# MrTornado24/IDE-3D

Measured on AMD Instinct MI355X. Metric: 512x512 RGB+seg frames/s @96 depth samples (whole job), higher is better.
Workload: dtype f32 (3x3 convs + MLPs: fp32 operands as 3 bf16 pieces, 6 products, f32 accumulate)

## Files before the change

### ide-3d_amd/csrc/modconv.hip

```cpp
#include "common.h"
#include "knobs.h"
#include <stdlib.h>
#include <string.h>
#include <type_traits>

namespace ide3d {

typedef float f32x16 __attribute__((ext_vector_type(16)));

#ifdef IDE3D_MC_TRACE
__device__ unsigned long long g_mc_dbg[256];
#define IDE3D_MC_TS(k) { const unsigned long long now_ = __builtin_readcyclecounter(); mc_acc[k] += now_ - mc_last; mc_last = now_; }
#else
#define IDE3D_MC_TS(k)
#endif

enum { MODE_CONV3 = 0, MODE_CONV1 = 1, MODE_TCONV3 = 2, MODE_TCONV3A = 3, MODE_CONV3S2 = 4 };

template <int MODE> struct ModeCfg;
template <> struct ModeCfg<MODE_CONV3>  { static constexpr int KC = 4, WTAPS = 9, MAXT = 9; };
template <> struct ModeCfg<MODE_CONV1>  { static constexpr int KC = 16, WTAPS = 1, MAXT = 1; };
template <> struct ModeCfg<MODE_CONV3S2> { static constexpr int KC = 4, WTAPS = 9, MAXT = 9; };
template <> struct ModeCfg<MODE_TCONV3> { static constexpr int KC = 4, WTAPS = 9, MAXT = 4; };
template <> struct ModeCfg<MODE_TCONV3A> { static constexpr int KC = 4, WTAPS = 9, MAXT = 9; };

template <int MODE, int BIG, int TI, int PH, int PW, int NWV = 4, int KCO = 0>
struct McCfg {
    static constexpr int NT = 64 * NWV;
    static constexpr int BN = TI * PH * PW;
    static_assert(BN == 64 || BN == 128 || BN == 256, "pixel tile must hold 64, 128 or 256 pixels");
    static constexpr int NCLS = (MODE == MODE_TCONV3A) ? 4 : 1;
    using MC = ModeCfg<MODE>;
    static constexpr int KC = KCO ? KCO : MC::KC, WTAPS = MC::WTAPS, MAXT = MC::MAXT;
    static constexpr int WM = BIG ? 2 : 1, WN = NWV / WM;
    static constexpr int MTW = (BIG == 1) ? 2 : 1;
    static constexpr int NTW = (BN / 32) / WN;
    static constexpr int BM = WM * MTW * 32;
    static constexpr int STRIDE = (MODE == MODE_CONV3S2) ? 2 : 1;
    static constexpr int HALO = (MODE == MODE_CONV1 || MODE == MODE_CONV3S2) ? 0 : 1;
    static constexpr int HP = (MODE == MODE_CONV3S2) ? 2 * PH + 1 : PH + 2 * HALO;
    static constexpr int HW = (MODE == MODE_CONV3S2) ? 2 * PW + 1 : PW + 2 * HALO;
    static constexpr int XW = (MODE == MODE_CONV1) ? PW : (MODE == MODE_CONV3S2) ? ((HW + 3) & ~3) : ((PW == 16) ? 48 : HW + 2);
    static constexpr int XS = HP * XW;
    static constexpr int XI = KC * XS;
    static constexpr int LDS_W = MAXT * KC * BM;
    static constexpr int LDS_X = TI * XI;
    static constexpr int NW4 = (LDS_W / 4 + NT - 1) / NT;
    static constexpr int VW = (MODE == MODE_CONV1 && PH == 1 && PW % 4 == 0) ? 4 : 1;
    static constexpr int NXE = (TI * KC * HP * HW / VW + NT - 1) / NT;
};

template <int N>
__device__ __forceinline__ int sel(const int (&a)[N], int t) {
    int v = a[0];
#pragma unroll
    for (int i = 1; i < N; ++i) v = (t == i) ? a[i] : v;
    return v;
}

__host__ __device__ inline int mc_bm(int cout) { return cout > 96 ? 128 : (cout > 32 ? 64 : 32); }
__host__ __device__ inline int mc_kc(int k) { return k == 3 ? 4 : 16; }

__global__ void __launch_bounds__(256)
modconv_pack_kernel(const float* __restrict__ w, int64_t w_batch_stride, int nbatch, int cout, int cin, int taps, int bm, int kc,
                    int mblocks, int cchunks, float* __restrict__ out) {
    const int64_t total = (int64_t)nbatch * mblocks * cchunks * taps * kc * bm;
    const int64_t stride = (int64_t)gridDim.x * blockDim.x;
    for (int64_t i = (int64_t)blockIdx.x * blockDim.x + threadIdx.x; i < total; i += stride) {
        int64_t r = i;
        const int co_l = (int)(r % bm); r /= bm;
        const int cil = (int)(r % kc); r /= kc;
        const int tap = (int)(r % taps); r /= taps;
        const int cc = (int)(r % cchunks); r /= cchunks;
        const int mb = (int)(r % mblocks); r /= mblocks;
        const int nb = (int)r;
        const int co = mb * bm + co_l, ci = cc * kc + cil;
        out[i] = (co < cout && ci < cin) ? w[nb * w_batch_stride + ((int64_t)co * cin + ci) * taps + tap] : 0.f;
    }
}

struct ConvGeom {
    int tiles_x[4], tiles_y[4];
    int tile_base[5];
    int img_groups;
    int mblocks, cchunks, split_k, chunks_per_split;
    int oh, ow;
    int debug;
};

template <int OFF_BYTES>
__device__ __forceinline__ float lds_read_async(unsigned addr) {
    float v;
    asm volatile("ds_read_b32 %0, %1 offset:%2" : "=v"(v) : "v"(addr), "n"(OFF_BYTES));
    return v;
}
template <int PENDING>
__device__ __forceinline__ void lds_wait(float& first) { asm volatile("s_waitcnt lgkmcnt(%1)" : "+v"(first) : "n"(PENDING)); }
__device__ __forceinline__ void lds_pin(float& v) { asm volatile("" : "+v"(v)); }
__device__ __forceinline__ unsigned lds_addr(const float* p) { return (unsigned)(size_t)p; }

template <class F, int... Is>
__device__ __forceinline__ void static_for_impl(F&& f, std::integer_sequence<int, Is...>) { (f(std::integral_constant<int, Is>{}), ...); }
template <int N, class F>
__device__ __forceinline__ void static_for(F&& f) { static_for_impl(f, std::make_integer_sequence<int, N>{}); }

template <int MODE, int XW>
__host__ __device__ constexpr int tap_patch_offset(int t) {
    return (MODE == MODE_CONV1) ? 0
         : (MODE == MODE_TCONV3A) ? ((t / 3 == 2) ? 0 : 1) * XW + ((t % 3 == 2) ? 0 : 1)
         : (t / 3) * XW + (t % 3);
}
template <int MODE>
__host__ __device__ constexpr int tap_class(int t) { return (MODE == MODE_TCONV3A) ? ((t / 3) & 1) * 2 + ((t % 3) & 1) : 0; }

__device__ __forceinline__ void amax_acc(float& m, float v) { m = fmaxf(m, fabsf(v)); }
__device__ __forceinline__ void amax_commit(float* y_amax, int n, float v, bool) {
    if (v > 0.f) amax_raise(y_amax, n, v);
}

template <int MODE, int TI, int PH, int PW, int NWV, int NCLS, int MTW, int NTW, int BM, int SCRATCH, int ROWPAR = -1>
__device__ __forceinline__ void modconv_finish(const ide3d_modconv_params& p, float* __restrict__ partial, const ConvGeom& g,
                                               f32x16 (&acc)[NCLS][MTW][NTW], float* s_w, int mb, int n0, int y0, int x0, int split, int cls,
                                               int wm, int wn, int lp, const float* __restrict__ row_unscale = nullptr, float x_unscale = 1.f,
                                               int team_tid = -1, float* amax_scratch = nullptr) {
    constexpr int NT = 64 * NWV;
    const int tid = team_tid >= 0 ? team_tid : (int)threadIdx.x, lane = tid & 63, wid = tid >> 6, half = lane >> 5;
    const int cpy = cls >> 1, cpx = cls & 1;
    const bool raw = (g.split_k > 1);
    float* const s_dm = s_w;
    float* const s_bi = s_w + TI * BM;
    for (int e = tid; e < TI * BM; e += NT) {
        const int rl = e % BM, co = mb * BM + rl, n = min(n0 + e / BM, p.n - 1);
        float d = (!raw && p.dcoefs && co < p.cout) ? p.dcoefs[(int64_t)n * p.cout + co] : 1.f;
        if (row_unscale) d *= row_unscale[co] * x_unscale;
        s_dm[e] = d;
        if (e < BM) s_bi[e] = (!raw && p.bias && co < p.cout) ? p.bias[co] : 0.f;
    }
    __syncthreads();
    float* const dst = raw ? partial + (int64_t)split * p.n * p.cout * g.oh * g.ow : p.y;
    const int64_t pitch = (!raw && p.y_pitch > 0) ? p.y_pitch : g.ow;
    const float e_alpha = (!raw && p.act == 3) ? p.alpha : 1.f, e_gain = raw ? 1.f : p.gain;
    const float e_clamp = (!raw && p.clamp >= 0.f) ? p.clamp : __builtin_inff();
    const float e_nstr = (!raw && p.noise) ? p.noise_strength : 0.f;
    auto finish = [&](float v, float d, float nz, float bb) {
        v *= d; v += nz; v += bb;
        v = (v > 0.f) ? v : v * e_alpha;
        v *= e_gain;
        return fminf(fmaxf(v, -e_clamp), e_clamp);
    };
    const bool want_amax = !raw && p.y_amax != nullptr;
    float amax_tile = 0.f;
    constexpr int QX = (MODE == MODE_TCONV3A) ? 2 : 1, QY = NCLS / QX;
    static_assert(ROWPAR < 0 || (MODE == MODE_TCONV3A && NCLS == 2), "one row parity = two column classes");
    constexpr int TW = 32 * QX, TP = TW + 8;
    constexpr int AVAIL = SCRATCH - (TI + 1) * BM;
    constexpr int RR = (MODE == MODE_TCONV3 || PW % 4 != 0) ? 0 : (AVAIL >= NWV * 32 * TP) ? 32 : (AVAIL >= NWV * 16 * TP) ? 16 : (AVAIL >= NWV * 8 * TP) ? 8 : 0;
    if constexpr (RR > 0) {
        typedef float f32x4u __attribute__((ext_vector_type(4), aligned(4)));
        float* const T = s_w + (TI + 1) * BM + wid * (RR * TP);
#pragma unroll
        for (int qy = 0; qy < QY; ++qy)
#pragma unroll
        for (int j = 0; j < NTW; ++j) {
            const int pbase = (wn * NTW + j) * 32;
            const int c4 = lane % (TW / 4), row0 = lane / (TW / 4);
            const int pix = pbase + (c4 * 4) / QX, ti = pix / (PH * PW), rem = pix % (PH * PW);
            const int n = n0 + ti, gy = y0 + rem / PW, gx = x0 + rem % PW;
            const int oy = (MODE == MODE_TCONV3A) ? 2 * gy + (ROWPAR >= 0 ? ROWPAR : qy) : gy, ox = (MODE == MODE_TCONV3A) ? 2 * gx : gx;
            const bool px_ok = n < p.n && oy < g.oh && ox < g.ow, full = ox + 3 < g.ow;
            const int64_t pofs = (int64_t)oy * pitch + ox, nofs = (int64_t)oy * g.ow + ox;
            f32x4u nz = {0.f, 0.f, 0.f, 0.f};
            if (e_nstr != 0.f && px_ok) {
                if (full) nz = *reinterpret_cast<const f32x4u*>(p.noise + nofs) * e_nstr;
                else for (int e = 0; e < 4; ++e) if (ox + e < g.ow) nz[e] = p.noise[nofs + e] * e_nstr;
            }
            float* const o_px = dst + (int64_t)n * p.cout * ((int64_t)g.oh * pitch) + pofs;
            float amax_j = 0.f;
#pragma unroll
            for (int i = 0; i < MTW; ++i)
#pragma unroll
            for (int g0 = 0; g0 < 4; g0 += RR / 8) {
#pragma unroll
                for (int qx = 0; qx < QX; ++qx)
#pragma unroll
                    for (int gg = 0; gg < RR / 8; ++gg)
#pragma unroll
                        for (int rr = 0; rr < 4; ++rr)
                            T[(gg * 8 + rr + 4 * half) * TP + lp * QX + qx] = acc[qy * QX + qx][i][j][(g0 + gg) * 4 + rr];
#pragma unroll
                for (int k = 0; k < RR * (TW / 4) / 64; ++k) {
                    const int rowl = row0 + k * (256 / TW);
                    f32x4u v4 = *reinterpret_cast<const f32x4u*>(T + rowl * TP + c4 * 4);
                    const int rl = (wm * MTW + i) * 32 + g0 * 8 + rowl, co = mb * BM + rl;
                    if (!px_ok || co >= p.cout) continue;
                    const float d = s_dm[ti * BM + rl], bb = s_bi[rl];
#pragma unroll
                    for (int e = 0; e < 4; ++e) v4[e] = finish(v4[e], d, nz[e], bb);
                    float* o = o_px + (int64_t)co * ((int64_t)g.oh * pitch);
                    if (full) {
                        *reinterpret_cast<f32x4u*>(o) = v4;
                        if (want_amax) { amax_acc(amax_j, v4[0]); amax_acc(amax_j, v4[1]); amax_acc(amax_j, v4[2]); amax_acc(amax_j, v4[3]); }
                    } else for (int e = 0; e < 4; ++e) if (ox + e < g.ow) { o[e] = v4[e]; amax_acc(amax_j, v4[e]); }
                }
            }
            if (want_amax) { if (TI == 1) amax_tile = fmaxf(amax_tile, amax_j); else if (px_ok) amax_commit(p.y_amax, n, amax_j, false); }
        }
    } else {
#pragma unroll
    for (int q = 0; q < NCLS; ++q)
#pragma unroll
    for (int j = 0; j < NTW; ++j) {
        const int pix = (wn * NTW + j) * 32 + lp;
        const int ti = pix / (PH * PW), rem = pix % (PH * PW);
        const int n = n0 + ti;
        const int gy = y0 + rem / PW, gx = x0 + rem % PW;
        const int oy = (MODE == MODE_TCONV3) ? 2 * gy + cpy : gy, ox = (MODE == MODE_TCONV3) ? 2 * gx + cpx : gx;
        const bool ok = n < p.n && oy < g.oh && ox < g.ow;
        if (!ok) continue;
        const float nz = (e_nstr != 0.f) ? p.noise[oy * g.ow + ox] * e_nstr : 0.f;
        float amax_j = 0.f;
#pragma unroll
        for (int i = 0; i < MTW; ++i)
#pragma unroll
            for (int r = 0; r < 16; ++r) {
                const int rl = (wm * MTW + i) * 32 + (r & 3) + 8 * (r >> 2) + 4 * half;
                const int co = mb * BM + rl;
                if (co >= p.cout) continue;
                const float v = finish(acc[q][i][j][r], s_dm[ti * BM + rl], nz, s_bi[rl]);
                *(dst + (((int64_t)n * p.cout + co) * g.oh + oy) * pitch + ox) = v;
                amax_acc(amax_j, v);
            }
        if (want_amax) { if (TI == 1) amax_tile = fmaxf(amax_tile, amax_j); else amax_commit(p.y_amax, n, amax_j, false); }
    }
    }
    if (TI == 1 && p.y_amax != nullptr && !raw && n0 < p.n)
        amax_raise_block(p.y_amax, n0, amax_tile, amax_scratch ? amax_scratch : s_w);
}

template <int MODE, int BIG, int TI, int PH, int PW, int NWV, int KCO>
__device__ __forceinline__ void modconv_tile(const ide3d_modconv_params& p, const float* __restrict__ wp, float* __restrict__ partial,
                                             const ConvGeom& g, float* s_w, float* s_x, int mb, int tl, int grp, int split, int cls,
                                             int tiles_x) {
    using K = McCfg<MODE, BIG, TI, PH, PW, NWV, KCO>;
#ifdef IDE3D_MC_TRACE
    const unsigned long long mc_t0 = __builtin_readcyclecounter();
#endif
    const int tid = threadIdx.x, lane = tid & 63, wid = tid >> 6;
    const int wm = wid / K::WN, wn = wid % K::WN;
    const int half = lane >> 5, l32 = lane & 31;
    const int txi = tl % tiles_x, tyi = tl / tiles_x;
    const int y0 = tyi * PH, x0 = txi * PW;
    const int n0 = grp * TI;
    const int cpy = cls >> 1, cpx = cls & 1;

    int ntaps, t_widx[K::MAXT], t_off[K::MAXT];
    if (MODE == MODE_CONV3 || MODE == MODE_CONV3S2) {
        ntaps = 9;
#pragma unroll
        for (int t = 0; t < 9; ++t) { t_widx[t] = t; t_off[t] = (t / 3) * K::XW + (t % 3); }
    } else if (MODE == MODE_CONV1) {
        ntaps = 1; t_widx[0] = 0; t_off[0] = 0;
    } else if (MODE == MODE_TCONV3A) {
        ntaps = 9;
#pragma unroll
        for (int t = 0; t < 9; ++t) {
            const int ky = t / 3, kx = t % 3;
            t_widx[t] = t; t_off[t] = ((ky == 2) ? 0 : 1) * K::XW + ((kx == 2) ? 0 : 1);
        }
    } else {
        const int nky = cpy ? 1 : 2, nkx = cpx ? 1 : 2;
        ntaps = nky * nkx;
#pragma unroll
        for (int t = 0; t < 4; ++t) {
            const int a = t / nkx, b = t % nkx;
            const int ky = cpy ? 1 : (a == 0 ? 0 : 2), kx = cpx ? 1 : (b == 0 ? 0 : 2);
            const int dy = (ky == 2) ? 0 : 1, dx = (kx == 2) ? 0 : 1;
            t_widx[t] = ky * 3 + kx; t_off[t] = dy * K::XW + dx;
        }
    }

    const float* __restrict__ wsrc = wp + (int64_t)mb * g.cchunks * (K::WTAPS * K::KC * K::BM)
                                     + (p.w_batch_stride ? (int64_t)n0 * g.mblocks * g.cchunks * (K::WTAPS * K::KC * K::BM) : 0);
    int x_src[K::NXE], x_dst[K::NXE], x_img[K::NXE];
#pragma unroll
    for (int i = 0; i < K::NXE; ++i) {
        const int e = tid + i * K::NT;
        x_src[i] = -1; x_dst[i] = -1; x_img[i] = 0;
        if (e < TI * K::KC * K::HP * K::HW / K::VW) {
            int r = e;
            const int rx = (r % (K::HW / K::VW)) * K::VW; r /= (K::HW / K::VW);
            const int ry = r % K::HP; r /= K::HP;
            const int cil = r % K::KC; r /= K::KC;
            const int ti = r;
            const int yy = y0 * K::STRIDE - K::HALO + ry, xx = x0 * K::STRIDE - K::HALO + rx;
            x_dst[i] = ti * K::XI + cil * K::XS + ry * K::XW + rx;
            x_img[i] = ti * K::KC + cil;
            if (n0 + ti < p.n && yy >= 0 && yy < p.h && xx >= 0 && xx < p.w_)
                x_src[i] = ((n0 + ti) * p.cin + cil) * (p.h * p.w_) + yy * p.w_ + xx;
        }
    }
    const int hw = p.h * p.w_;

    f32x16 acc[K::NCLS][K::MTW][K::NTW];
#pragma unroll
    for (int q = 0; q < K::NCLS; ++q)
#pragma unroll
        for (int i = 0; i < K::MTW; ++i)
#pragma unroll
            for (int j = 0; j < K::NTW; ++j)
#pragma unroll
                for (int r = 0; r < 16; ++r) acc[q][i][j][r] = 0.f;

    int boff[K::NTW];
#pragma unroll
    for (int j = 0; j < K::NTW; ++j) {
        const int pix = (wn * K::NTW + j) * 32 + l32;
        const int ti = pix / (PH * PW), rem = pix % (PH * PW);
        boff[j] = ti * K::XI + (rem / PW) * K::STRIDE * K::XW + (rem % PW) * K::STRIDE + half * K::XS;
    }
    const int aoff = half * K::BM + wm * K::MTW * 32 + l32;

    const int c_begin = split * g.chunks_per_split;
    const int c_end = min(c_begin + g.chunks_per_split, g.cchunks);

    typedef float f32x4v __attribute__((ext_vector_type(4)));
    using XV = std::conditional_t<K::VW == 4, f32x4v, float>;
    XV xreg[K::NXE];
    float sreg[K::NXE];
    const int img_last = p.n - 1;
    constexpr int PIECE = (K::KC * K::BM < 256) ? K::KC * K::BM : 256;
    constexpr int PPT = K::KC * K::BM / PIECE;
    const int w_pieces = ntaps * PPT;
#ifdef IDE3D_MC_TRACE
    unsigned long long mc_acc[6] = {0, 0, 0, 0, 0, 0}, mc_last = 0;
#endif
    auto fetch = [&](int c, int buf) {
        const float* ws = wsrc + (int64_t)c * (K::WTAPS * K::KC * K::BM);
        for (int i = wid; i < w_pieces; i += NWV) {
            const int t = i / PPT, r = (i - t * PPT) * PIECE;
            const float* src = ws + ((MODE == MODE_TCONV3) ? sel(t_widx, t) : t) * (K::KC * K::BM) + r + lane * 4;
            if (lane * 4 < PIECE)
                __builtin_amdgcn_global_load_lds((const __attribute__((address_space(1))) void*)src,
                                                 (__attribute__((address_space(3))) void*)(s_w + buf * K::LDS_W + t * (K::KC * K::BM) + r), 16, 0, 0);
        }
        IDE3D_MC_TS(5)
        const int ci0 = c * K::KC;
#pragma unroll
        for (int i = 0; i < K::NXE; ++i) {
            const int cil = x_img[i] % K::KC;
            const int ci = min(ci0 + cil, p.cin - 1);
            const int64_t src = (x_src[i] >= 0) ? (int64_t)x_src[i] + (int64_t)(ci - cil) * hw : 0;
            xreg[i] = *reinterpret_cast<const XV*>(p.x + src);
            sreg[i] = p.styles ? p.styles[min(n0 + x_img[i] / K::KC, img_last) * p.cin + ci] : 1.0f;
        }
    };
    auto commit = [&](int buf, int c) {
        const int ci0 = c * K::KC;
#pragma unroll
        for (int i = 0; i < K::NXE; ++i) {
            const int cil = x_img[i] % K::KC;
            const bool live = x_src[i] >= 0 && ci0 + cil < p.cin;
            XV v = xreg[i] * sreg[i];
            if (!live) __builtin_memset(&v, 0, sizeof(v));
            if (x_dst[i] >= 0) *reinterpret_cast<XV*>(s_x + buf * K::LDS_X + x_dst[i]) = v;
        }
    };

    if (c_begin < c_end) {
        fetch(c_begin, 0);
        commit(0, c_begin);
    }
    __syncthreads();
#ifdef IDE3D_MC_TRACE
    mc_last = __builtin_readcyclecounter();
    const unsigned long long mc_prologue = mc_last - mc_t0;
#endif
    for (int c = c_begin; c < c_end; ++c) {
        const int buf = (c - c_begin) & 1;
        IDE3D_MC_TS(0)
        if (c + 1 < c_end && g.debug != 1) fetch(c + 1, buf ^ 1);
        IDE3D_MC_TS(1)
        const float* sw = s_w + buf * K::LDS_W;
        const float* sx = s_x + buf * K::LDS_X;
        auto tap_body = [&](int t, int off, auto cls_tag) {
            constexpr int q = decltype(cls_tag)::value;
#pragma unroll
            for (int cp = 0; cp < K::KC / 2; ++cp) {
                float a[K::MTW], b[K::NTW];
#pragma unroll
                for (int i = 0; i < K::MTW; ++i) a[i] = sw[(t * K::KC + cp * 2) * K::BM + aoff + i * 32];
#pragma unroll
                for (int j = 0; j < K::NTW; ++j) b[j] = sx[boff[j] + cp * 2 * K::XS + off];
#pragma unroll
                for (int i = 0; i < K::MTW; ++i)
#pragma unroll
                    for (int j = 0; j < K::NTW; ++j)
                        acc[q][i][j] = __builtin_amdgcn_mfma_f32_32x32x2f32(a[i], b[j], acc[q][i][j], 0, 0, 0);
            }
        };
        using C0 = std::integral_constant<int, 0>;
        if constexpr (MODE == MODE_TCONV3) {
            for (int t = 0; t < ntaps; ++t) tap_body(t, sel(t_off, t), C0{});
        } else {
            constexpr int KP = K::KC / 2, G = 2, SPT = KP / G, NSTEP = K::MAXT * SPT, NRD = G * (K::MTW + K::NTW);
            static_assert(KP % G == 0 && NRD <= 15, "lgkmcnt is a 4-bit counter");
            const unsigned a_base = lds_addr(sw + aoff);
            unsigned b_base[K::NTW];
#pragma unroll
            for (int j = 0; j < K::NTW; ++j) b_base[j] = lds_addr(sx + boff[j]);
            float av[2][G][K::MTW], bv[2][G][K::NTW];
            auto issue = [&](auto ss) {
                constexpr int S = decltype(ss)::value, T = S / SPT, CP0 = (S % SPT) * G, B = S & 1;
                static_for<G>([&](auto cc) {
                    constexpr int CP = CP0 + decltype(cc)::value, CI = decltype(cc)::value;
                    static_for<K::MTW>([&](auto ii) {
                        constexpr int I = decltype(ii)::value;
                        av[B][CI][I] = lds_read_async<((T * K::KC + CP * 2) * K::BM + I * 32) * 4>(a_base);
                    });
                    static_for<K::NTW>([&](auto jj) {
                        constexpr int J = decltype(jj)::value;
                        bv[B][CI][J] = lds_read_async<(CP * 2 * K::XS + tap_patch_offset<MODE, K::XW>(T)) * 4>(b_base[J]);
                    });
                });
            };
            issue(C0{});
            static_for<NSTEP>([&](auto ss) {
                constexpr int S = decltype(ss)::value, B = S & 1, Q = tap_class<MODE>(S / SPT);
                if constexpr (S + 1 < NSTEP) issue(std::integral_constant<int, S + 1>{});
                lds_wait<(S + 1 < NSTEP) ? NRD : 0>(av[B][0][0]);
#pragma unroll
                for (int cp = 0; cp < G; ++cp) {
#pragma unroll
                    for (int i = 0; i < K::MTW; ++i) lds_pin(av[B][cp][i]);
#pragma unroll
                    for (int j = 0; j < K::NTW; ++j) lds_pin(bv[B][cp][j]);
                }
#pragma unroll
                for (int cp = 0; cp < G; ++cp)
#pragma unroll
                    for (int i = 0; i < K::MTW; ++i)
#pragma unroll
                        for (int j = 0; j < K::NTW; ++j)
                            acc[Q][i][j] = __builtin_amdgcn_mfma_f32_32x32x2f32(av[B][cp][i], bv[B][cp][j], acc[Q][i][j], 0, 0, 0);
            });
        }
        IDE3D_MC_TS(2)
        if (c + 1 < c_end && g.debug != 1) commit(buf ^ 1, c + 1);
        asm volatile("s_waitcnt vmcnt(0)" ::: "memory");
        IDE3D_MC_TS(3)
        if (g.debug != 1) __syncthreads();
        IDE3D_MC_TS(4)
    }

#ifdef IDE3D_MC_TRACE
    const unsigned long long mc_t1 = __builtin_readcyclecounter();
#endif
    modconv_finish<MODE, TI, PH, PW, NWV, K::NCLS, K::MTW, K::NTW, K::BM, 2 * K::LDS_W>(p, partial, g, acc, s_w, mb, n0, y0, x0, split, cls, wm, wn, l32);
#ifdef IDE3D_MC_TRACE
    if (blockIdx.x == 100 && threadIdx.x == 0) {
        for (int k = 0; k < 6; ++k) g_mc_dbg[k] = mc_acc[k];
        g_mc_dbg[7] = (unsigned long long)(c_end - c_begin);
        g_mc_dbg[8] = mc_prologue;
        g_mc_dbg[9] = __builtin_readcyclecounter() - mc_t1;
    }
#endif
}


typedef unsigned u32x4 __attribute__((ext_vector_type(4)));
typedef unsigned u32x2 __attribute__((ext_vector_type(2)));
typedef __bf16 bf16x8 __attribute__((ext_vector_type(8)));
typedef __bf16 bf16x2 __attribute__((ext_vector_type(2)));
typedef float f32x2 __attribute__((ext_vector_type(2)));

template <int MODE, int BIG, int PH, int PARTS, int WBUF = 2, int NWV_ = 4, int PAIR = 0>
struct SpCfg {
    static_assert(MODE == MODE_CONV3 || MODE == MODE_TCONV3A, "split-bf16 loop: 3x3 and all-class transposed 3x3 only");
    static_assert(BIG == 1 || BIG == 2, "64- or 128-row blocks");
    static_assert(NWV_ == 4 || NWV_ == 8, "4 or 8 waves");
    static constexpr int PW = 16, NWV = NWV_, NT = 64 * NWV;
    static constexpr int BN = PH * PW;
    static_assert(!PAIR || MODE == MODE_TCONV3A, "row-parity pairs exist in the transposed form only");
    static constexpr int NCLS = (MODE == MODE_TCONV3A) ? (PAIR ? 2 : 4) : 1;
    static constexpr int BM = (BIG == 1) ? 128 : 64;
    static constexpr int WM = (BIG == 2 && PH == 32) ? 1 : 2, WN = NWV / WM;
    static constexpr int MTW = BM / 32 / WM, NTW = BN / 32 / WN;
    static_assert(MTW >= 1 && MTW * 32 * WM == BM, "row block must split into 32-row MFMA tiles per wave");
    static_assert(NTW >= 1 && NTW * 32 * WN == BN, "pixel tile must split into 32-pixel MFMA tiles per wave");
    static constexpr int NLOAD = 4;
    static constexpr int KC = 16;
    static constexpr int HALO = (MODE == MODE_TCONV3A) ? 1 : 2;
    static constexpr int HP = PH + HALO, HW = PW + HALO, NSLOT = HP * HW;
    static constexpr int NS = PARTS * (PARTS + 1) / 2;
    static constexpr int W_UNITS = 3 * PARTS * 2 * BM;
    static constexpr int X_UNITS = PARTS * 2 * NSLOT;
    static constexpr int NXR = (NSLOT + 63) / 64;
    static constexpr int LDS_BYTES = 16 * (WBUF * W_UNITS + 2 * X_UNITS);
    static_assert(LDS_BYTES <= 160 * 1024, "LDS of one CU");
};

__host__ __device__ inline int64_t sp_packed_units(int mblocks, int cchunks, int bm, int parts) { return (int64_t)mblocks * cchunks * 9 * parts * 2 * bm; }

__device__ __forceinline__ unsigned pk_bf16(float a, float b) {
    f32x2 v = {a, b};
    return __builtin_bit_cast(unsigned, __builtin_convertvector(v, bf16x2));
}
typedef _Float16 f16x2 __attribute__((ext_vector_type(2)));
typedef _Float16 f16x8 __attribute__((ext_vector_type(8)));
template <int PARTS, int F16 = 0>
__device__ __forceinline__ void split_pair(float a, float b, unsigned (&out)[PARTS]) {
    if constexpr (F16) {
        static_assert(PARTS == 2, "the fp16 split has two pieces");
        const f32x2 v = {a, b};
        const unsigned hi = __builtin_bit_cast(unsigned, __builtin_convertvector(v, f16x2));
        f32x2 r;
        asm("v_fma_mix_f32 %0, %1, -1.0, %2 op_sel_hi:[1,0,0]" : "=v"(r.x) : "v"(hi), "v"(a));
        asm("v_fma_mix_f32 %0, %1, -1.0, %2 op_sel:[1,0,0] op_sel_hi:[1,0,0]" : "=v"(r.y) : "v"(hi), "v"(b));
        out[0] = hi; out[1] = __builtin_bit_cast(unsigned, __builtin_convertvector(r, f16x2));
    } else {
#pragma unroll
    for (int q = 0; q < PARTS; ++q) {
        const unsigned pk = pk_bf16(a, b);
        out[q] = pk;
        if (q + 1 < PARTS) { a -= __uint_as_float(pk << 16); b -= __uint_as_float(pk & 0xffff0000u); }
    }
    }
}
template <int F16>
__device__ __forceinline__ f32x16 sp_mfma(const u32x4& a, const u32x4& b, const f32x16& c) {
    if constexpr (F16) return __builtin_amdgcn_mfma_f32_32x32x16_f16(__builtin_bit_cast(f16x8, a), __builtin_bit_cast(f16x8, b), c, 0, 0, 0);
    else return __builtin_amdgcn_mfma_f32_32x32x16_bf16(__builtin_bit_cast(bf16x8, a), __builtin_bit_cast(bf16x8, b), c, 0, 0, 0);
}
__device__ __forceinline__ void f16_scale(float bound, float& scale, float& unscale) {
    scale = 1.f; unscale = 1.f;
    if (bound > 0.f && bound < __builtin_inff()) {
        int e;
        frexpf(bound, &e);
        e = min(max(15 - e, -126), 126);
        scale = ldexpf(1.f, e); unscale = ldexpf(1.f, -e);
    }
}

__global__ void __launch_bounds__(256)
modconv_row_scale_kernel(const float* __restrict__ w, int cout, int rowlen, int rows_padded, float* __restrict__ scale, float* __restrict__ unscale) {
    const int row = blockIdx.x * 4 + (threadIdx.x >> 6), lane = threadIdx.x & 63;
    if (row >= rows_padded) return;
    float m = 0.f;
    if (row < cout) for (int i = lane; i < rowlen; i += 64) m = fmaxf(m, fabsf(w[(int64_t)row * rowlen + i]));
#pragma unroll
    for (int off = 32; off > 0; off >>= 1) m = fmaxf(m, __shfl_xor(m, off));
    if (lane == 0) { float sc, us; f16_scale(m, sc, us); scale[row] = sc; unscale[row] = us; }
}

template <int PARTS, int F16 = 0>
__global__ void __launch_bounds__(256)
modconv_pack_split_kernel(const float* __restrict__ w, int cout, int cin, int bm, int mblocks, int cchunks, u32x4* __restrict__ out,
                          const float* __restrict__ row_scale = nullptr) {
    const int64_t total = (int64_t)mblocks * cchunks * 9 * 2 * bm;
    const int64_t stride = (int64_t)gridDim.x * blockDim.x;
    for (int64_t i = (int64_t)blockIdx.x * blockDim.x + threadIdx.x; i < total; i += stride) {
        int64_t r = i;
        const int co_l = (int)(r % bm); r /= bm;
        const int kg = (int)(r % 2); r /= 2;
        const int tap = (int)(r % 9); r /= 9;
        const int cc = (int)(r % cchunks); r /= cchunks;
        const int mb = (int)r;
        const int co = mb * bm + co_l;
        const float rs = F16 ? row_scale[co] : 1.f;
        unsigned pk[4][PARTS];
#pragma unroll
        for (int e = 0; e < 4; ++e) {
            const int ci = cc * 16 + kg * 8 + e * 2;
            const float a = (co < cout && ci < cin) ? w[((int64_t)co * cin + ci) * 9 + tap] * rs : 0.f;
            const float b = (co < cout && ci + 1 < cin) ? w[((int64_t)co * cin + ci + 1) * 9 + tap] * rs : 0.f;
            split_pair<PARTS, F16>(a, b, pk[e]);
        }
        const int64_t base = (((int64_t)(mb * cchunks + cc) * 9 + tap) * PARTS * 2 + kg) * bm + co_l;
#pragma unroll
        for (int q = 0; q < PARTS; ++q) {
            const u32x4 v = {pk[0][q], pk[1][q], pk[2][q], pk[3][q]};
            out[base + (int64_t)q * 2 * bm] = v;
        }
    }
}

template <int OFF_BYTES>
__device__ __forceinline__ u32x4 lds_read128_async(unsigned addr) {
    u32x4 v;
    asm volatile("ds_read_b128 %0, %1 offset:%2" : "=v"(v) : "v"(addr), "n"(OFF_BYTES));
    return v;
}
template <int PENDING>
__device__ __forceinline__ void lds_wait128(u32x4& first) { asm volatile("s_waitcnt lgkmcnt(%1)" : "+v"(first) : "n"(PENDING)); }
__device__ __forceinline__ void lds_pin128(u32x4& v) { asm volatile("" : "+v"(v)); }

template <int MODE, int BIG, int PH, int PARTS, int WBUF, int NWV, int F16, int TEAMS = 1, int PAR = -1>
__device__ __forceinline__ void modconv_split_tile(const ide3d_modconv_params& p, const u32x4* __restrict__ wp, float* __restrict__ partial,
                                                   const ConvGeom& g, unsigned char* smem, int mb, int tl, int grp, int split, int tiles_x,
                                                   const float* __restrict__ row_unscale, float* wg_scratch = nullptr) {
    using K = SpCfg<MODE, BIG, PH, PARTS, WBUF, NWV, (PAR >= 0)>;
    static_assert(!F16 || PARTS == 2, "f16x3 = two fp16 pieces per operand");
    static_assert(PAR < 0 || (MODE == MODE_TCONV3A && WBUF == 2 && TEAMS == 1), "row-parity pairs: transposed form, two weight buffers, one team");
    constexpr int NST = (PAR < 0) ? 3 : (PAR == 0 ? 2 : 1);
    auto kys = [](int i) constexpr { return (PAR < 0) ? i : (PAR == 0 ? 2 * i : 1); };
    static_assert(TEAMS == 1 || (TEAMS == 2 && NWV == 4), "two teams of four waves, or one team");
    constexpr int PW = K::PW;
    const int tid = (TEAMS == 2) ? (int)(threadIdx.x & 255u) : (int)threadIdx.x, lane = tid & 63;
    const int wid = __builtin_amdgcn_readfirstlane(tid >> 6);
    const int wm = wid / K::WN, wn = wid % K::WN;
    const int half = lane >> 5, l32 = lane & 31;
    const int lp = ((((l32 >> 2) ^ (l32 >> 3) ^ (l32 >> 4)) & 1) << 4) | (l32 & 15);
    const int txi = tl % tiles_x, tyi = tl / tiles_x;
    const int y0 = tyi * PH, x0 = txi * PW;
    const int n0 = grp;
    u32x4* const s_w = reinterpret_cast<u32x4*>(smem);
    u32x4* const s_x = s_w + WBUF * K::W_UNITS;

    f32x16 acc[K::NCLS][K::MTW][K::NTW];
#pragma unroll
    for (int q = 0; q < K::NCLS; ++q)
#pragma unroll
        for (int i = 0; i < K::MTW; ++i)
#pragma unroll
            for (int j = 0; j < K::NTW; ++j)
#pragma unroll
                for (int r = 0; r < 16; ++r) acc[q][i][j][r] = 0.f;

    const int hw = p.h * p.w_;
    int x_src[K::NXR];
#pragma unroll
    for (int r = 0; r < K::NXR; ++r) {
        const int sidx = lane + 64 * r;
        const int ry = sidx / K::HW, rx = sidx % K::HW;
        const int yy = y0 - 1 + ry, xx = x0 - 1 + rx;
        x_src[r] = (sidx < K::NSLOT && yy >= 0 && yy < p.h && xx >= 0 && xx < p.w_) ? yy * p.w_ + xx : -1;
    }
    const float* __restrict__ ximg = p.x + (int64_t)n0 * p.cin * hw;
    float xreg[K::NXR][4];
    float sty[4];
    float xs = 1.f, xus = 1.f;
    if constexpr (F16) {
        float mm = p.styles ? 0.f : 1.f;
        if (p.styles) for (int ci = lane; ci < p.cin; ci += 64) mm = fmaxf(mm, fabsf(p.styles[(int64_t)n0 * p.cin + ci]));
        float xm = (lane < IDE3D_AMAX_SLOTS) ? p.x_amax[(int64_t)n0 * IDE3D_AMAX_FLOATS + lane * IDE3D_AMAX_STRIDE] : 0.f;
#pragma unroll
        for (int off = 32; off > 0; off >>= 1) { mm = fmaxf(mm, __shfl_xor(mm, off)); xm = fmaxf(xm, __shfl_xor(xm, off)); }
        f16_scale(mm * xm, xs, xus);
    }
    const bool stages_patch = (NWV == 4) || wid < 4;
    auto fetch_patch = [&](int c) {
        if (!stages_patch) return;
        const int ci0 = c * K::KC + wid * 4;
#pragma unroll
        for (int k = 0; k < 4; ++k) {
            const int ci = min(ci0 + k, p.cin - 1);
            sty[k] = (ci0 + k < p.cin) ? (p.styles ? p.styles[(int64_t)n0 * p.cin + ci] : 1.f) : 0.f;
#pragma unroll
            for (int r = 0; r < K::NXR; ++r) xreg[r][k] = ximg[(int64_t)ci * hw + max(x_src[r], 0)];
        }
    };
    auto commit_patch = [&](int buf) {
        if (!stages_patch) return;
        unsigned char* const dst = reinterpret_cast<unsigned char*>(s_x + buf * K::X_UNITS) + ((wid >> 1) * K::NSLOT) * 16 + (wid & 1) * 8;
        const float sc[4] = {F16 ? sty[0] * xs : sty[0], F16 ? sty[1] * xs : sty[1], F16 ? sty[2] * xs : sty[2], F16 ? sty[3] * xs : sty[3]};
#pragma unroll
        for (int r = 0; r < K::NXR; ++r) {
            const int sidx = lane + 64 * r;
            const bool live = x_src[r] >= 0;
            unsigned lo[PARTS], hi[PARTS];
            split_pair<PARTS, F16>(live ? xreg[r][0] * sc[0] : 0.f, live ? xreg[r][1] * sc[1] : 0.f, lo);
            split_pair<PARTS, F16>(live ? xreg[r][2] * sc[2] : 0.f, live ? xreg[r][3] * sc[3] : 0.f, hi);
            if (sidx < K::NSLOT) {
#pragma unroll
                for (int q = 0; q < PARTS; ++q) {
                    const u32x2 v = {lo[q], hi[q]};
                    *reinterpret_cast<u32x2*>(dst + (q * 2 * K::NSLOT + sidx) * 16) = v;
                }
            }
        }
    };
    const u32x4* __restrict__ wsrc = wp + (int64_t)mb * g.cchunks * 3 * K::W_UNITS;
    constexpr int W_PIECES = K::W_UNITS / 64;
    static_assert(K::W_UNITS % 64 == 0, "weight stage is a whole number of 1 KB pieces");
    constexpr int W_COL = (W_PIECES + 3) / 4;
    constexpr int W_EARLY = (NWV == 8) ? (W_COL * 5 + 8) / 9 : W_COL;
    auto fetch_weights = [&](int stage, int buf, bool late = false) {
        const u32x4* src = wsrc + (int64_t)stage * K::W_UNITS;
        if (NWV == 4 && late) return;
        if (NWV == 8 && (late != (wid < 4))) return;
        const int m0 = late ? W_EARLY : 0, m1 = late ? W_COL : W_EARLY;
        for (int m = m0; m < m1; ++m) {
            const int i = (wid & 3) + 4 * m;
            if (i < W_PIECES)
                __builtin_amdgcn_global_load_lds((const __attribute__((address_space(1))) void*)(src + i * 64 + lane),
                                                 (__attribute__((address_space(3))) void*)(s_w + buf * K::W_UNITS + i * 64), 16, 0, 0);
        }
    };

    const unsigned a_base0 = (unsigned)(size_t)(s_w + half * K::BM + wm * K::MTW * 32 + l32);
    unsigned b_base0[K::NTW];
#pragma unroll
    for (int j = 0; j < K::NTW; ++j) {
        const int pix = (wn * K::NTW + j) * 32 + lp;
        b_base0[j] = (unsigned)(size_t)(s_x + half * K::NSLOT + (pix / PW) * K::HW + (pix % PW));
    }

    const int c_begin = split * g.chunks_per_split;
    const int c_end = min(c_begin + g.chunks_per_split, g.cchunks);
#ifdef IDE3D_MC_TRACE
    unsigned long long mc_acc[6] = {0, 0, 0, 0, 0, 0}, mc_last = 0;
    const unsigned long long mc_t0 = __builtin_readcyclecounter();
#endif
    if (c_begin < c_end) {
        if (WBUF == 2) { fetch_weights(c_begin * 3 + kys(0), 0); if (NWV == 8) fetch_weights(c_begin * 3 + kys(0), 0, true); }
        fetch_patch(c_begin);
        commit_patch(0);
    }
    asm volatile("s_waitcnt vmcnt(0)" ::: "memory");
    __syncthreads();
    int wbuf = 0;
#ifdef IDE3D_MC_TRACE
    mc_last = __builtin_readcyclecounter();
    const unsigned long long mc_prologue = mc_last - mc_t0;
#endif
    for (int c = c_begin; c < c_end; ++c) {
        const int xbuf = (c - c_begin) & 1;
        const bool more = c + 1 < c_end;
        static_for<NST>([&](auto sii) {
            constexpr int SI = decltype(sii)::value, KY = kys(SI);
            constexpr bool LAST = (SI == NST - 1), MID = (SI == (NST == 3 ? 1 : 0));
            const int next_stage = LAST ? (c + 1) * 3 + kys(0) : c * 3 + kys(LAST ? 0 : SI + 1);
            IDE3D_MC_TS(0)
            if constexpr (WBUF == 2) {
                if (!LAST || more) fetch_weights(next_stage, wbuf ^ 1);
                if (MID && more) fetch_patch(c + 1);
            } else {
                fetch_weights(c * 3 + KY, 0);
                if (MID && more) fetch_patch(c + 1);
                asm volatile("s_waitcnt vmcnt(0)" ::: "memory");
                __syncthreads();
            }
            IDE3D_MC_TS(1)
            const unsigned a_base = a_base0 + ((WBUF == 2) ? wbuf * (K::W_UNITS * 16) : 0);
            unsigned b_base[K::NTW];
#pragma unroll
            for (int j = 0; j < K::NTW; ++j) b_base[j] = b_base0[j] + xbuf * (K::X_UNITS * 16);
            constexpr int GRP = K::MTW + K::NTW, NGRP = 3 * PARTS;
            constexpr int SP_AHEAD = 1;
            constexpr int NBUF = (PARTS == 2 && SP_AHEAD > 1) ? 3 : 2;
            constexpr int AHEAD_CAP = 15 / GRP - 1, AHEAD_SAFE = (NBUF - 1) * PARTS - 1;
            constexpr int AHEAD = (SP_AHEAD < AHEAD_CAP ? SP_AHEAD : AHEAD_CAP) < AHEAD_SAFE ? (SP_AHEAD < AHEAD_CAP ? SP_AHEAD : AHEAD_CAP) : AHEAD_SAFE;
            static_assert(AHEAD >= 1 && (AHEAD + 1) * GRP <= 15, "lgkmcnt is a 4-bit counter");
            constexpr bool B_REUSE = (MODE == MODE_TCONV3A) && NBUF == 2;
            u32x4 av[NBUF][K::MTW][PARTS], bv[NBUF][K::NTW][PARTS];
            auto issue = [&](auto ss) {
                constexpr int S = decltype(ss)::value, KX = S / PARTS, Q = S % PARTS, B = KX % NBUF, T = KY * 3 + KX;
                constexpr int BS = B_REUSE ? (KX == 2 ? 1 : 0) : B;
                static_for<K::MTW>([&](auto ii) {
                    constexpr int I = decltype(ii)::value;
                    av[B][I][Q] = lds_read128_async<(((KX * PARTS + Q) * 2) * K::BM + I * 32) * 16>(a_base);
                });
                if constexpr (!(B_REUSE && KX == 1))
                static_for<K::NTW>([&](auto jj) {
                    constexpr int J = decltype(jj)::value;
                    bv[BS][J][Q] = lds_read128_async<(Q * 2 * K::NSLOT + tap_patch_offset<MODE, K::HW>(T)) * 16>(b_base[J]);
                });
            };
            static_for<AHEAD>([&](auto ss) { issue(ss); });
            static_for<NGRP>([&](auto ss) {
                constexpr int S = decltype(ss)::value, KX = S / PARTS, Q = S % PARTS, B = KX % NBUF, QC = (PAR >= 0) ? (KX & 1) : tap_class<MODE>(KY * 3 + KX);
                constexpr int BS = B_REUSE ? (KX == 2 ? 1 : 0) : B;
                if constexpr (S + AHEAD < NGRP) issue(std::integral_constant<int, S + AHEAD>{});
                constexpr int PENDING = [] { int n = 0; for (int s2 = S + 1; s2 <= S + AHEAD && s2 < NGRP; ++s2) n += K::MTW + ((B_REUSE && s2 / PARTS == 1) ? 0 : K::NTW); return n; }();
                lds_wait128<PENDING>(av[B][0][Q]);
#pragma unroll
                for (int i = 0; i < K::MTW; ++i) lds_pin128(av[B][i][Q]);
                if constexpr (!(B_REUSE && KX == 1)) {
#pragma unroll
                for (int j = 0; j < K::NTW; ++j) lds_pin128(bv[BS][j][Q]);
                }
#pragma unroll
                for (int qa = 0; qa <= Q; ++qa)
#pragma unroll
                    for (int qb = 0; qb <= Q; ++qb) {
                        if ((qa == Q || qb == Q) && qa + qb < PARTS) {
#pragma unroll
                            for (int i = 0; i < K::MTW; ++i)
#pragma unroll
                                for (int j = 0; j < K::NTW; ++j)
                                    acc[QC][i][j] = sp_mfma<F16>(av[B][i][qa], bv[BS][j][qb], acc[QC][i][j]);
                        }
                    }
            });
            IDE3D_MC_TS(2)
            if (LAST && more) commit_patch(xbuf ^ 1);
            if constexpr (WBUF == 2 && NWV == 8) { if (!LAST || more) fetch_weights(next_stage, wbuf ^ 1, true); }
            IDE3D_MC_TS(3)
            if (WBUF == 2) asm volatile("s_waitcnt vmcnt(0)" ::: "memory");
            IDE3D_MC_TS(4)
            __syncthreads();
            IDE3D_MC_TS(5)
            wbuf ^= 1;
        });
    }
#ifdef IDE3D_MC_TRACE
    const unsigned long long mc_t1 = __builtin_readcyclecounter();
#endif
    modconv_finish<MODE, 1, PH, PW, K::NWV, K::NCLS, K::MTW, K::NTW, K::BM, K::LDS_BYTES / 4, PAR>(p, partial, g, acc, reinterpret_cast<float*>(smem), mb, n0, y0, x0, split, 0, wm, wn, lp,
                                                                                                F16 ? row_unscale : nullptr, xus, (TEAMS == 2) ? tid : -1, wg_scratch);
#ifdef IDE3D_MC_TRACE
    if (blockIdx.x == 100 && (threadIdx.x == 0 || threadIdx.x == 256)) {
        const int o = threadIdx.x ? 16 : 0;
        for (int k = 0; k < 6; ++k) g_mc_dbg[o + k] = mc_acc[k];
        g_mc_dbg[o + 7] = (unsigned long long)(c_end - c_begin) * 3;
        g_mc_dbg[o + 8] = mc_prologue;
        g_mc_dbg[o + 9] = __builtin_readcyclecounter() - mc_t1;
    }
#endif
}



constexpr int head_waves(int mt) { return mt == 1 ? 16 : 8; }
template <int PARTS, int MT>
struct HeadCfg {
    static constexpr int ROWS = MT * 32;
    static constexpr int A_UNITS = PARTS * 2 * ROWS;
    static constexpr int NWV = head_waves(MT);
    static constexpr int BN = 32 * NWV;
};
__host__ __device__ inline int64_t head_packed_units(int n, int cchunks, int parts, int mt) { return (int64_t)n * cchunks * parts * 2 * mt * 32; }

template <int PARTS>
__global__ void __launch_bounds__(256)
head_pack_split_kernel(const float* __restrict__ w, int64_t w_batch_stride, int n, int cout, int cin, int rows, int cchunks, u32x4* __restrict__ out) {
    const int64_t total = (int64_t)n * cchunks * 2 * rows;
    const int64_t stride = (int64_t)gridDim.x * blockDim.x;
    for (int64_t i = (int64_t)blockIdx.x * blockDim.x + threadIdx.x; i < total; i += stride) {
        int64_t r = i;
        const int row = (int)(r % rows); r /= rows;
        const int kg = (int)(r % 2); r /= 2;
        const int cc = (int)(r % cchunks); r /= cchunks;
        const int nb = (int)r;
        unsigned pk[4][PARTS];
#pragma unroll
        for (int e = 0; e < 4; ++e) {
            const int ci = cc * 16 + kg * 8 + e * 2;
            const float a = (row < cout && ci < cin) ? w[nb * w_batch_stride + (int64_t)row * cin + ci] : 0.f;
            const float b = (row < cout && ci + 1 < cin) ? w[nb * w_batch_stride + (int64_t)row * cin + ci + 1] : 0.f;
            split_pair<PARTS>(a, b, pk[e]);
        }
        const int64_t base = (((int64_t)nb * cchunks + cc) * PARTS * 2 + kg) * rows + row;
#pragma unroll
        for (int q = 0; q < PARTS; ++q) {
            const u32x4 v = {pk[0][q], pk[1][q], pk[2][q], pk[3][q]};
            out[base + (int64_t)q * 2 * rows] = v;
        }
    }
}

template <int PARTS, int MT>
__global__ void __launch_bounds__(64 * head_waves(MT), head_waves(MT) / 4)
head_split_kernel(ide3d_modconv_params p, const u32x4* __restrict__ wp, int cchunks, int tiles_per_image) {
    using K = HeadCfg<PARTS, MT>;
    if constexpr (K::NWV == 16) asm volatile("" ::: "v127"); else asm volatile("" ::: "v255");
    constexpr int S_MIN = K::NWV * 32 * 40 / 4 + 2 * K::ROWS / 4 + 16;
    constexpr int S_UNITS = (2 * K::A_UNITS > S_MIN) ? 2 * K::A_UNITS : S_MIN;
    __shared__ __attribute__((aligned(16))) u32x4 s_a[S_UNITS];
    const int tid = threadIdx.x, lane = tid & 63, half = lane >> 5, l32 = lane & 31;
    const int wid = __builtin_amdgcn_readfirstlane(tid >> 6);
    const int bid = xcd_remap(blockIdx.x, gridDim.x);
    const int n0 = bid / tiles_per_image, tile = bid % tiles_per_image;
    const int hw = p.h * p.w_;
    const int pix = tile * K::BN + wid * 32 + l32;
    const int pix_c = min(pix, hw - 1);
    const float* __restrict__ xl = p.x + (int64_t)n0 * p.cin * hw + (int64_t)(8 * half) * hw + pix_c;
    const u32x4* __restrict__ wsrc = wp + (int64_t)n0 * cchunks * K::A_UNITS;

    f32x16 acc[1][MT][1];
#pragma unroll
    for (int m = 0; m < MT; ++m)
#pragma unroll
        for (int r = 0; r < 16; ++r) acc[0][m][0][r] = 0.f;

    constexpr int A_PIECES = K::A_UNITS / 64;
    static_assert(K::A_UNITS % 64 == 0, "whole 1 KB pieces");
    auto fetch_a = [&](int c, int buf) {
        for (int i = wid; i < A_PIECES; i += K::NWV)
            __builtin_amdgcn_global_load_lds((const __attribute__((address_space(1))) void*)(wsrc + (int64_t)c * K::A_UNITS + i * 64 + lane),
                                             (__attribute__((address_space(3))) void*)(s_a + buf * K::A_UNITS + i * 64), 16, 0, 0);
    };
    float xr[3][8];
    auto fetch_b = [&](int c, auto slot_tag) {
        constexpr int SLOT = decltype(slot_tag)::value;
#pragma unroll
        for (int e = 0; e < 8; ++e) {
            const int ch = c * 16 + 8 * half + e;
            const float v = xl[(int64_t)(min(ch, p.cin - 1) - 8 * half) * hw];
            xr[SLOT][e] = (ch < p.cin) ? v : 0.f;
        }
    };
    using S0 = std::integral_constant<int, 0>; using S1 = std::integral_constant<int, 1>; using S2 = std::integral_constant<int, 2>;
    fetch_a(0, 0); fetch_b(0, S0{});
    if (cchunks > 1) fetch_b(1, S1{});
    auto chunk = [&](int c, auto slot_tag) {
        constexpr int SLOT = decltype(slot_tag)::value, NSLOT = (SLOT + 2) % 3;
        if (c + 1 < cchunks) asm volatile("s_waitcnt vmcnt(8)" ::: "memory"); else asm volatile("s_waitcnt vmcnt(0)" ::: "memory");
        __syncthreads();
        if (c + 1 < cchunks) fetch_a(c + 1, (c + 1) & 1);
        if (c + 2 < cchunks) fetch_b(c + 2, std::integral_constant<int, NSLOT>{});
        u32x4 bfrag[PARTS];
        {
            unsigned pk[4][PARTS];
#pragma unroll
            for (int e = 0; e < 4; ++e) split_pair<PARTS>(xr[SLOT][2 * e], xr[SLOT][2 * e + 1], pk[e]);
#pragma unroll
            for (int q = 0; q < PARTS; ++q) bfrag[q] = u32x4{pk[0][q], pk[1][q], pk[2][q], pk[3][q]};
        }
        const u32x4* sa = s_a + (c & 1) * K::A_UNITS + half * K::ROWS + l32;
#pragma unroll
        for (int m = 0; m < MT; ++m) {
            u32x4 af[PARTS];
#pragma unroll
            for (int q = 0; q < PARTS; ++q) af[q] = sa[q * 2 * K::ROWS + m * 32];
#pragma unroll
            for (int qa = 0; qa < PARTS; ++qa)
#pragma unroll
                for (int qb = 0; qa + qb < PARTS; ++qb)
                    acc[0][m][0] = __builtin_amdgcn_mfma_f32_32x32x16_bf16(__builtin_bit_cast(bf16x8, af[qa]), __builtin_bit_cast(bf16x8, bfrag[qb]), acc[0][m][0], 0, 0, 0);
        }
    };
    for (int c = 0; c < cchunks; c += 3) {
        chunk(c, S0{});
        if (c + 1 < cchunks) chunk(c + 1, S1{});
        if (c + 2 < cchunks) chunk(c + 2, S2{});
    }
    __syncthreads();
    ide3d_modconv_params pf = p;
    pf.h = 1; pf.w_ = hw;
    ConvGeom g{};
    g.oh = 1; g.ow = hw; g.split_k = 1;
    modconv_finish<MODE_CONV1, 1, 1, K::BN, K::NWV, 1, MT, 1, K::ROWS, S_UNITS * 4>(pf, nullptr, g, acc, reinterpret_cast<float*>(s_a), 0, n0, 0, tile * K::BN, 0, 0, 0, wid, l32);
}


template <class T>
__device__ __forceinline__ T* uniform_ptr(T* ptr) {
    const uint64_t v = reinterpret_cast<uint64_t>(ptr);
    const unsigned lo = __builtin_amdgcn_readfirstlane((unsigned)v), hi = __builtin_amdgcn_readfirstlane((unsigned)(v >> 32));
    return reinterpret_cast<T*>(((uint64_t)hi << 32) | lo);
}
template <int PARTS, int MT, int NCH>
__global__ void __launch_bounds__(512, 2)
head_resident_kernel(ide3d_modconv_params p, const u32x4* __restrict__ wp, int wgs_per_image, int tiles32) {
    using K = HeadCfg<PARTS, MT>;
    asm volatile("" ::: "v255");
    constexpr int NWV = 8, NBUF = (MT == 1) ? 2 : 1;
    __shared__ __attribute__((aligned(16))) u32x4 s_a[NCH * K::A_UNITS + K::ROWS / 4 + 4];
    float* const s_bi = reinterpret_cast<float*>(s_a + NCH * K::A_UNITS);
    const int tid = threadIdx.x, lane = tid & 63, half = lane >> 5, l32 = lane & 31;
    const int wid = __builtin_amdgcn_readfirstlane(tid >> 6);
    const int n0 = blockIdx.x % p.n, slot = blockIdx.x / p.n;
// ... 957 lines not shown
```

Before: 900.5.

## Use 16x16x32 bf16 MFMA tiles for three-piece fp32 emulated 3x3 convs

For the three-bf16-piece 3x3 conv path, the inner loop switches from 32x32 MFMA tiles to 16x16x32 bf16 MFMAs. It adds new LDS addressing with a permuted pixel mapping, so the six cross products are packed as three K=32 instructions per tap. The epilogue gains a 16x16 C-layout staging path. The aim is more product work per MFMA and fewer LDS reads per step. In exchange it holds more accumulator registers and uses complex lane permutations, which risks register pressure and correctness.

Measured after the change: 907.3 (median of 6 runs). No clear change (+0.8%).

```diff
diff --git a/ide-3d_amd/csrc/modconv.hip b/ide-3d_amd/csrc/modconv.hip
--- a/ide-3d_amd/csrc/modconv.hip
+++ b/ide-3d_amd/csrc/modconv.hip
@@ -118,9 +118,9 @@
     if (v > 0.f) amax_raise(y_amax, n, v);
 }
 
-template <int MODE, int TI, int PH, int PW, int NWV, int NCLS, int MTW, int NTW, int BM, int SCRATCH, int ROWPAR = -1>
+template <int MODE, int TI, int PH, int PW, int NWV, int NCLS, int MTW, int NTW, int BM, int SCRATCH, int ROWPAR = -1, int C16 = 0, class ACC>
 __device__ __forceinline__ void modconv_finish(const ide3d_modconv_params& p, float* __restrict__ partial, const ConvGeom& g,
-                                               f32x16 (&acc)[NCLS][MTW][NTW], float* s_w, int mb, int n0, int y0, int x0, int split, int cls,
+                                               ACC& acc, float* s_w, int mb, int n0, int y0, int x0, int split, int cls,
                                                int wm, int wn, int lp, const float* __restrict__ row_unscale = nullptr, float x_unscale = 1.f,
                                                int team_tid = -1, float* amax_scratch = nullptr) {
     constexpr int NT = 64 * NWV;
@@ -155,6 +155,7 @@
     constexpr int TW = 32 * QX, TP = TW + 8;
     constexpr int AVAIL = SCRATCH - (TI + 1) * BM;
     constexpr int RR = (MODE == MODE_TCONV3 || PW % 4 != 0) ? 0 : (AVAIL >= NWV * 32 * TP) ? 32 : (AVAIL >= NWV * 16 * TP) ? 16 : (AVAIL >= NWV * 8 * TP) ? 8 : 0;
+    static_assert(!C16 || RR >= 16, "the 16 x 16 C layout is staged 16 rows (one row of C tiles) at a time");
     if constexpr (RR > 0) {
         typedef float f32x4u __attribute__((ext_vector_type(4), aligned(4)));
         float* const T = s_w + (TI + 1) * BM + wid * (RR * TP);
@@ -181,12 +182,23 @@
 #pragma unroll
             for (int g0 = 0; g0 < 4; g0 += RR / 8) {
 #pragma unroll
-                for (int qx = 0; qx < QX; ++qx)
+                for (int qx = 0; qx < QX; ++qx) {
+                    if constexpr (C16) {
+#pragma unroll
+                        for (int si = 0; si < RR / 16; ++si)
+#pragma unroll
+                            for (int sj = 0; sj < 2; ++sj)
+#pragma unroll
+                                for (int rr = 0; rr < 4; ++rr)
+                                    T[(si * 16 + 4 * (lane >> 4) + rr) * TP + (sj * 16 + lp) * QX + qx] = acc[qy * QX + qx][2 * i + g0 / 2 + si][2 * j + sj][rr];
+                    } else {
 #pragma unroll
                     for (int gg = 0; gg < RR / 8; ++gg)
 #pragma unroll
                         for (int rr = 0; rr < 4; ++rr)
                             T[(gg * 8 + rr + 4 * half) * TP + lp * QX + qx] = acc[qy * QX + qx][i][j][(g0 + gg) * 4 + rr];
+                    }
+                }
 #pragma unroll
                 for (int k = 0; k < RR * (TW / 4) / 64; ++k) {
                     const int rowl = row0 + k * (256 / TW);
@@ -492,6 +504,7 @@
     static constexpr int HALO = (MODE == MODE_TCONV3A) ? 1 : 2;
     static constexpr int HP = PH + HALO, HW = PW + HALO, NSLOT = HP * HW;
     static constexpr int NS = PARTS * (PARTS + 1) / 2;
+    static constexpr bool MF16 = (PARTS == 3 && MODE == MODE_CONV3);
     static constexpr int W_UNITS = 3 * PARTS * 2 * BM;
     static constexpr int X_UNITS = PARTS * 2 * NSLOT;
     static constexpr int NXR = (NSLOT + 63) / 64;
@@ -525,6 +538,10 @@
         if (q + 1 < PARTS) { a -= __uint_as_float(pk << 16); b -= __uint_as_float(pk & 0xffff0000u); }
     }
     }
+}
+typedef float f32x4 __attribute__((ext_vector_type(4)));
+__device__ __forceinline__ f32x4 sp_mfma16(const u32x4& a, const u32x4& b, const f32x4& c) {
+    return __builtin_amdgcn_mfma_f32_16x16x32_bf16(__builtin_bit_cast(bf16x8, a), __builtin_bit_cast(bf16x8, b), c, 0, 0, 0);
 }
 template <int F16>
 __device__ __forceinline__ f32x16 sp_mfma(const u32x4& a, const u32x4& b, const f32x16& c) {
@@ -625,6 +642,14 @@
             for (int j = 0; j < K::NTW; ++j)
 #pragma unroll
                 for (int r = 0; r < 16; ++r) acc[q][i][j][r] = 0.f;
+    constexpr int MT16 = K::MF16 ? 2 * K::MTW : 1, NT16 = K::MF16 ? 2 * K::NTW : 1;
+    f32x4 acc16[K::NCLS][MT16][NT16];
+#pragma unroll
+    for (int q = 0; q < K::NCLS; ++q)
+#pragma unroll
+        for (int i = 0; i < MT16; ++i)
+#pragma unroll
+            for (int j = 0; j < NT16; ++j) acc16[q][i][j] = f32x4{0.f, 0.f, 0.f, 0.f};
 
     const int hw = p.h * p.w_;
     int x_src[K::NXR];
@@ -704,6 +729,12 @@
         const int pix = (wn * K::NTW + j) * 32 + lp;
         b_base0[j] = (unsigned)(size_t)(s_x + half * K::NSLOT + (pix / PW) * K::HW + (pix % PW));
     }
+    const int sel = (lane >> 4) & 1, c16 = lane & 15;
+    const int pp = (c16 & 9) | (((c16 >> 1) & 1) << 2) | ((1 ^ (c16 >> 2) ^ (c16 >> 3)) & 1) << 1;
+    const unsigned a01_base0 = (unsigned)(size_t)(s_w + (sel * 2 + half) * K::BM + wm * K::MTW * 32 + c16);
+    const unsigned a02_base0 = (unsigned)(size_t)(s_w + (sel * 4 + half) * K::BM + wm * K::MTW * 32 + c16);
+    const unsigned b00_base0 = (unsigned)(size_t)(s_x + half * K::NSLOT + (wn * NT16) * K::HW + pp);
+    const unsigned b20_base0 = (unsigned)(size_t)(s_x + ((1 - sel) * 4 + half) * K::NSLOT + (wn * NT16) * K::HW + pp);
 
     const int c_begin = split * g.chunks_per_split;
     const int c_end = min(c_begin + g.chunks_per_split, g.cchunks);
@@ -741,6 +772,59 @@
                 __syncthreads();
             }
             IDE3D_MC_TS(1)
+            if constexpr (K::MF16) {
+            static_assert(PARTS == 3 && !F16, "16x16x32 pairing: three bf16 pieces");
+            constexpr bool B_REUSE = (MODE == MODE_TCONV3A);
+            constexpr int NSTEP = 9;
+            constexpr int BS_BYTES = 2 * K::NSLOT * 16;
+            const unsigned wofs = (WBUF == 2) ? wbuf * (K::W_UNITS * 16) : 0, xofs = xbuf * (K::X_UNITS * 16);
+            const unsigned a01b = a01_base0 + wofs, a02b = a02_base0 + wofs, b00b = b00_base0 + xofs, b20b = b20_base0 + xofs;
+            u32x4 a01[2][MT16], a02[2][MT16], b00[2][NT16], b11[2][NT16], b20[2][NT16];
+            auto n_reads = [](int s) constexpr {
+                const int kx = s / 3, m = s % 3;
+                return (m == 1 ? 0 : MT16) + ((B_REUSE && kx == 1) ? 0 : NT16);
+            };
+            auto issue = [&](auto ss) {
+                constexpr int S = decltype(ss)::value, KX = S / 3, M = S % 3, BA = KX & 1, BB = B_REUSE ? (KX == 2 ? 1 : 0) : (KX & 1);
+                constexpr int T = KY * 3 + KX, TOFS = tap_patch_offset<MODE, K::HW>(T) * 16;
+                static_for<MT16>([&](auto ii) {
+                    constexpr int I = decltype(ii)::value, AOFS = ((KX * PARTS * 2) * K::BM + I * 16) * 16;
+                    if constexpr (M == 0) a01[BA][I] = lds_read128_async<AOFS>(a01b);
+                    if constexpr (M == 2) a02[BA][I] = lds_read128_async<AOFS>(a02b);
+                });
+                if constexpr (!(B_REUSE && KX == 1))
+                static_for<NT16>([&](auto jj) {
+                    constexpr int J = decltype(jj)::value, BOFS = TOFS + J * K::HW * 16;
+                    if constexpr (M == 0) b00[BB][J] = lds_read128_async<BOFS>(b00b);
+                    if constexpr (M == 1) b11[BB][J] = lds_read128_async<BOFS + BS_BYTES>(b00b);
+                    if constexpr (M == 2) b20[BB][J] = lds_read128_async<BOFS>(b20b);
+                });
+            };
+            issue(std::integral_constant<int, 0>{});
+            static_for<NSTEP>([&](auto ss) {
+                constexpr int S = decltype(ss)::value, KX = S / 3, M = S % 3, BA = KX & 1, BB = B_REUSE ? (KX == 2 ? 1 : 0) : (KX & 1);
+                constexpr int QC = (PAR >= 0) ? (KX & 1) : tap_class<MODE>(KY * 3 + KX);
+                constexpr bool NEXT = S + 1 < NSTEP, EARLY = NEXT && n_reads(S) + n_reads(S + 1) <= 15;
+                static_assert(n_reads(S) <= 15, "lgkmcnt is a 4-bit counter");
+                if constexpr (EARLY) issue(std::integral_constant<int, S + 1>{});
+                if constexpr (n_reads(S) > 0) {
+                    u32x4& first = (M == 1) ? b11[BB][0] : (M == 0 ? a01[BA][0] : a02[BA][0]);
+                    lds_wait128<EARLY ? n_reads(S + 1) : 0>(first);
+#pragma unroll
+                    for (int i = 0; i < MT16; ++i) { if (M == 0) lds_pin128(a01[BA][i]); if (M == 2) lds_pin128(a02[BA][i]); }
+                    if constexpr (!(B_REUSE && KX == 1)) {
+#pragma unroll
+                    for (int j = 0; j < NT16; ++j) { if (M == 0) lds_pin128(b00[BB][j]); if (M == 1) lds_pin128(b11[BB][j]); if (M == 2) lds_pin128(b20[BB][j]); }
+                    }
+                }
+                if constexpr (NEXT && !EARLY) issue(std::integral_constant<int, S + 1>{});
+#pragma unroll
+                for (int i = 0; i < MT16; ++i)
+#pragma unroll
+                    for (int j = 0; j < NT16; ++j)
+                        acc16[QC][i][j] = sp_mfma16(M == 2 ? a02[BA][i] : a01[BA][i], M == 0 ? b00[BB][j] : (M == 1 ? b11[BB][j] : b20[BB][j]), acc16[QC][i][j]);
+            });
+            } else {
             const unsigned a_base = a_base0 + ((WBUF == 2) ? wbuf * (K::W_UNITS * 16) : 0);
             unsigned b_base[K::NTW];
 #pragma unroll
@@ -792,6 +876,7 @@
                         }
                     }
             });
+            }
             IDE3D_MC_TS(2)
             if (LAST && more) commit_patch(xbuf ^ 1);
             if constexpr (WBUF == 2 && NWV == 8) { if (!LAST || more) fetch_weights(next_stage, wbuf ^ 1, true); }
@@ -806,8 +891,12 @@
 #ifdef IDE3D_MC_TRACE
     const unsigned long long mc_t1 = __builtin_readcyclecounter();
 #endif
-    modconv_finish<MODE, 1, PH, PW, K::NWV, K::NCLS, K::MTW, K::NTW, K::BM, K::LDS_BYTES / 4, PAR>(p, partial, g, acc, reinterpret_cast<float*>(smem), mb, n0, y0, x0, split, 0, wm, wn, lp,
-                                                                                                F16 ? row_unscale : nullptr, xus, (TEAMS == 2) ? tid : -1, wg_scratch);
+    if constexpr (K::MF16)
+        modconv_finish<MODE, 1, PH, PW, K::NWV, K::NCLS, K::MTW, K::NTW, K::BM, K::LDS_BYTES / 4, PAR, 1>(p, partial, g, acc16, reinterpret_cast<float*>(smem), mb, n0, y0, x0, split, 0, wm, wn, pp,
+                                                                                                   F16 ? row_unscale : nullptr, xus, (TEAMS == 2) ? tid : -1, wg_scratch);
+    else
+        modconv_finish<MODE, 1, PH, PW, K::NWV, K::NCLS, K::MTW, K::NTW, K::BM, K::LDS_BYTES / 4, PAR, 0>(p, partial, g, acc, reinterpret_cast<float*>(smem), mb, n0, y0, x0, split, 0, wm, wn, lp,
+                                                                                                   F16 ? row_unscale : nullptr, xus, (TEAMS == 2) ? tid : -1, wg_scratch);
 #ifdef IDE3D_MC_TRACE
     if (blockIdx.x == 100 && (threadIdx.x == 0 || threadIdx.x == 256)) {
         const int o = threadIdx.x ? 16 : 0;
```
